# razvanmatisan/duodiff

Measured on AMD Instinct MI355X. Metric: images/sec (whole node) DuoDiff 1000-step CelebA-64, higher is better.
Workload: dtype bf16

## Files before the change

duodiff_amd/_lib.py:

```python
import ctypes as C
import os
from pathlib import Path

LIB_PATH = Path(os.environ.get("DUODIFF_LIB") or Path(__file__).resolve().parent / "libduodiff.so")

DD_OK = 0
DD_ERR_INVALID, DD_ERR_NOT_FOUND, DD_ERR_STATE, DD_ERR_HIP, DD_ERR_NOMEM, DD_ERR_UNSUPPORTED = -1, -2, -3, -4, -5, -6
DD_PREC_BF16, DD_PREC_FP32 = 0, 1
DD_VAR_BETA_TILDE, DD_VAR_BETA = 0, 1
DD_NOISE_NONE, DD_NOISE_BUFFER, DD_NOISE_PHILOX = 0, 1, 2
DD_X0_STATIC, DD_X0_DYNAMIC = 0, 1
DD_EE_MLP_PER_LAYER, DD_EE_MLP_PER_TIMESTEP, DD_EE_MLP_PER_LAYER_PER_TIMESTEP, DD_EE_ATTENTION_PROBE = 0, 1, 2, 3
ABI_VERSION = 6
DD_DEV_NO_FUSED_MLP, DD_DEV_NO_FUSED_PROJ, DD_DEV_NO_FUSED_HEAD, DD_DEV_GENERIC_EMBED, DD_DEV_MLP_EXTRAS_ONLY = 1, 2, 4, 8, 16
DD_DEV_NO_FUSED_SKIP, DD_DEV_NO_FUSED_QKV, DD_DEV_NO_FUSED_QA = 32, 64, 128
DD_PROF_DOMINANT, DD_PROF_BLOCK_TAIL, DD_PROF_FC1, DD_PROF_ROWLIN, DD_PROF_QKV_ATTENTION, DD_PROF_SPLITK = 0, 1, 2, 3, 4, 5
DD_DEV_NO_CHAINS, DD_DEV_FORCE_CHAINS, DD_DEV_NO_ROWLIN, DD_DEV_NO_ROWLIN_PROJ, DD_DEV_NO_EMBED_LN, DD_DEV_NO_SPLITK, DD_DEV_NO_ROWLIN_SKIP = 256, 512, 1024, 2048, 4096, 8192, 16384
DD_DEV_NO_SPLIT_HEADS = 32768
DD_DEV_NO_FRAG_AO, DD_DEV_NO_FRAG_SKIP, DD_DEV_NO_FRAG_X = 65536, 131072, 262144


class dd_config(C.Structure):
    _fields_ = [(n, C.c_int32) for n in (
        "img_size", "patch_size", "in_chans", "embed_dim", "depth", "num_heads", "mlp_ratio",
# ... 110 lines not shown
    "dd_bench_gemm": (C.c_int, [C.c_void_p, C.c_void_p, C.c_int, C.c_int, C.c_void_p, C.POINTER(C.c_float), C.POINTER(C.c_double)]),
    "dd_vae_create": (C.c_int, [C.c_void_p, C.c_int, C.c_int, C.POINTER(C.c_void_p)]),
    "dd_vae_set_param": (C.c_int, [C.c_void_p, C.c_char_p, C.c_void_p, C.POINTER(C.c_int64), C.c_int]),
    "dd_vae_finalize": (C.c_int, [C.c_void_p, C.c_int]),
    "dd_vae_decode": (C.c_int, [C.c_void_p, C.c_void_p, C.c_void_p, C.c_void_p, C.c_int, C.c_int, C.c_void_p]),
    "dd_vae_destroy": (None, [C.c_void_p]),
    "dd_vae_has_encoder": (C.c_int, [C.c_void_p]),
    "dd_vae_encode": (C.c_int, [C.c_void_p, C.c_void_p, C.c_void_p, C.c_void_p, C.c_void_p, C.c_void_p, C.c_int, C.c_int, C.c_void_p]),
    "dd_vae_sample": (C.c_int, [C.c_void_p, C.c_void_p, C.c_void_p, C.c_void_p, C.c_int, C.c_int, C.c_void_p]),
    "dd_profile_steps": (C.c_int, [C.c_void_p, C.c_void_p, C.c_void_p, C.c_void_p, C.c_int, C.c_int, C.c_int, C.c_void_p,
                                   C.POINTER(C.c_float), C.POINTER(C.c_int)]),
    "dd_profile_steps_chained": (C.c_int, [C.c_void_p, C.c_void_p, C.c_void_p, C.c_void_p, C.c_int, C.c_int, C.c_int, C.c_void_p,
                                           C.POINTER(C.c_float), C.POINTER(C.c_int)]),
    "dd_profile_select": (C.c_int, [C.c_void_p, C.c_int]),
    "dd_dev_qkv_attention": (C.c_int, [C.c_void_p, C.c_int, C.c_int, C.c_int, C.c_int, C.c_void_p, C.c_void_p, C.c_void_p, C.c_void_p,
                                       C.c_int, C.c_void_p, C.POINTER(C.c_float)]),
    "dd_dev_qkv_attention_rows": (C.c_int, [C.c_void_p, C.c_int, C.c_int, C.c_int, C.c_int] + [C.c_void_p] * 6 + [C.c_int, C.c_void_p, C.POINTER(C.c_float)]),
    "dd_dev_v_identity": (C.c_int, [C.c_void_p, C.c_int, C.c_int, C.c_int, C.c_int] + [C.c_void_p] * 6 + [C.c_int, C.c_void_p, C.POINTER(C.c_float)]),
    "dd_dev_v_copy": (C.c_int, [C.c_void_p] + [C.c_int] * 4 + [C.c_void_p] * 2 + [C.c_int, C.c_void_p, C.POINTER(C.c_float)]),
    "dd_dev_mlp": (C.c_int, [C.c_void_p, C.c_int, C.c_int, C.c_int, C.c_int] + [C.c_void_p] * 10 + [C.c_int, C.c_void_p, C.POINTER(C.c_float)] + [C.c_void_p] * 8),
    "dd_dev_block_tail": (C.c_int, [C.c_void_p] + [C.c_int] * 7 + [C.c_void_p] * 21 + [C.c_int, C.c_void_p, C.c_int, C.c_void_p, C.POINTER(C.c_float)]),
    "dd_dev_block_tail_frag": (C.c_int, [C.c_void_p] + [C.c_int] * 7 + [C.c_void_p] * 21 + [C.c_int, C.c_void_p, C.c_int, C.c_void_p, C.POINTER(C.c_float)] + [C.c_void_p] * 5),
    "dd_dev_qkv_attention_frag": (C.c_int, [C.c_void_p, C.c_int, C.c_int, C.c_int, C.c_int] + [C.c_void_p] * 7 + [C.c_int, C.c_void_p, C.POINTER(C.c_float)]),
    "dd_dev_head_dec": (C.c_int, [C.c_void_p] + [C.c_int] * 5 + [C.c_void_p] * 9 + [C.c_int, C.c_int, C.c_void_p, C.POINTER(C.c_float)]),
    "dd_dev_gemm": (C.c_int, [C.c_void_p] + [C.c_int] * 5 + [C.c_void_p] * 4 + [C.c_int] * 6 + [C.c_void_p] + [C.c_int] * 2 + [C.c_void_p] * 2 +
                    [C.c_int] + [C.c_void_p] * 3 + [C.c_int, C.c_int, C.c_void_p, C.POINTER(C.c_float)]),
    "dd_dev_rowlin": (C.c_int, [C.c_void_p] + [C.c_int] * 6 + [C.c_void_p] * 5 + [C.c_void_p] * 3 + [C.c_int, C.c_int, C.c_void_p, C.POINTER(C.c_float)]),
    "dd_dev_attention": (C.c_int, [C.c_void_p] + [C.c_int] * 4 + [C.c_void_p] * 4 + [C.c_int, C.c_void_p, C.POINTER(C.c_float)]),
    "dd_dev_layernorm": (C.c_int, [C.c_void_p] + [C.c_int] * 3 + [C.c_void_p] * 4 + [C.c_int] * 3 + [C.c_void_p, C.POINTER(C.c_float)]),
    "dd_dev_embed": (C.c_int, [C.c_void_p] + [C.c_int] * 9 + [C.c_void_p] * 7 + [C.c_float] + [C.c_void_p] * 3 + [C.c_int, C.c_void_p, C.POINTER(C.c_float)]),
    "dd_dev_time_mlp": (C.c_int, [C.c_void_p] + [C.c_int] * 5 + [C.c_void_p] * 6 + [C.c_float, C.c_void_p, C.c_int, C.c_void_p, C.POINTER(C.c_float)]),
    "dd_dev_vae_gather": (C.c_int, [C.c_void_p] + [C.c_int] * 6 + [C.c_void_p, C.c_void_p, C.c_size_t, C.c_void_p]),
    "dd_dev_poison_workspaces": (C.c_int, [C.c_void_p, C.c_void_p, C.c_void_p]),
    "dd_dev_graph_captures": (C.c_longlong, [C.c_void_p]),
    "dd_dev_last_sample_chains": (C.c_int, [C.c_void_p]),
    "dd_dev_set_flags": (C.c_int, [C.c_void_p, C.c_uint]),
    "dd_set_num_cus": (C.c_int, [C.c_void_p, C.c_int]),
    "dd_plan_rows": (C.c_int, [C.c_int, C.c_int, C.c_int, C.c_int, C.POINTER(C.c_int), C.POINTER(C.c_int)]),
    "dd_last_sample_timing": (C.c_int, [C.c_void_p, C.POINTER(C.c_float)]),
}

_lib = None


class EngineUnavailable(RuntimeError):
    """libduodiff.so is missing or unusable.  There is no CPU path to fall back to."""
# ... 29 lines not shown
```

duodiff_amd/csrc/attention.hip:

```cpp
#include "dd_internal.h"
#include "wave_prims.h"

#include <type_traits>
#include <utility>

namespace dd {
namespace {

constexpr int kMaxKeyTiles = 9;
constexpr int kLP = kMaxKeyTiles * 32;
constexpr int kHD = 64;
constexpr int kPartBytes = 4 * 2 * 66 * 4;

__device__ __forceinline__ int k_swz(int r) { return ((r >> 1) & 7) ^ ((r & 1) << 2); }
__device__ __forceinline__ int v_swz(int r) { return (2 * (r & 3)) ^ ((r >> 2) & 1); }

template <typename T> struct AttnLayout;
template <> struct AttnLayout<bf16_t> {
    static constexpr int kRowK = 128;
    static constexpr int kRowV = 128;
    static constexpr int kVBytes = kLP * kRowV;
};
template <> struct AttnLayout<float> {
    static constexpr int kRowK = 256 + 16;
// ... 313 lines not shown
                float f;
                if constexpr (sizeof(T) == 2) f = __builtin_amdgcn_exp2f((m[w] - M) * (0.125f * 1.4426950408889634f));
                else f = expf((m[w] - M) * 0.125f);
                num = fmaf(f, part[(w * 2 + qi) * 66 + d], num);
                den = fmaf(f, part[(w * 2 + qi) * 66 + 65], den);
            }
            out[((long long)b * L + 256 + qi) * D + hh * kHD + d] = Elem<T>::from_f32(num / den);
        }
    }
}


struct QkvAttnArgs {
    const bf16_t* h;
    const bf16_t* wimg;
    const float* bias;
    const bf16_t* hx;
    const float* xres;
    const float* ln_g;
    const float* ln_b;
    bf16_t* out;
    int B, L, H, Lp, E;
    bf16_t* out_frag = nullptr;
};

constexpr int kQaPxBytes = 8 * 6 * 2 * 32 * 4;
constexpr int kQaHxPad = 64;
constexpr int kQaHxBytes = 2 * (1024 * 2 + kQaHxPad);
constexpr int kQaAuxBytes = kQaPxBytes + kQaHxBytes + 256;
constexpr int kQaKQ = 8;
constexpr int kQaBlk = 2 * kQaKQ * 1024;
constexpr int kQaRing = 4 * kQaBlk;
static_assert(8 * 2 * 66 * 4 <= kQaPxBytes, "the split chunk's partials reuse the px area");

constexpr int qa_dma_ops(int b, int nb) { return b < nb ? 2 : 0; }
constexpr int qa_pref_ops(int b, int nb) { return (b >= 0 && b % 3 == 0 && b / 3 + 1 < nb / 3) ? kQaKQ : 0; }
constexpr int qa_younger_dma(int b, int nb) { return qa_pref_ops(b - 1, nb) + qa_dma_ops(b + 2, nb) + qa_pref_ops(b, nb); }
constexpr int qa_younger_rows(int b, int nb) { return qa_dma_ops(b, nb) + qa_dma_ops(b + 1, nb) + qa_dma_ops(b + 2, nb); }

template <int D>
__global__ void __launch_bounds__(512, 1) qkv_attention_kernel(const QkvAttnArgs a) {
    using Lay = AttnLayout<bf16_t>;
    constexpr int KS = D / 16, NS = KS / kQaKQ, NB = 3 * NS;
    static_assert(D % 128 == 0 && D >= 512 && D <= 1024, "k range in slices of 8 k-steps; hxl holds two rows of D <= 1024");
    extern __shared__ __attribute__((aligned(16))) char smem[];
    char* Ks = smem;
    char* Vt = smem + kLP * Lay::kRowK;
    float* px = reinterpret_cast<float*>(smem + kLP * Lay::kRowK + Lay::kVBytes);
    float* part = px;
    char* hxl = smem + kLP * Lay::kRowK + Lay::kVBytes + kQaPxBytes;
    char* qxl = hxl + kQaHxBytes;
    char* ring = smem + kLP * Lay::kRowK + Lay::kVBytes + kQaAuxBytes;

    int b, hh;
    if ((a.B & 7) == 0) { const int slot = blockIdx.x >> 3; b = (blockIdx.x & 7) + 8 * (slot / a.H); hh = slot % a.H; }
    else { b = blockIdx.x / a.H; hh = blockIdx.x % a.H; }
    const int tid = threadIdx.x, lane = tid & 63, wave = __builtin_amdgcn_readfirstlane(tid >> 6);
    const int half = lane >> 5, r32 = lane & 31;
    const int L = a.L, E = a.E;

    const char* wsrc = reinterpret_cast<const char*>(a.wimg) + (size_t)hh * NB * kQaBlk;
    const unsigned lane16 = lane * 16;
    auto dma_block = [&](int bb) {
#pragma unroll
        for (int i = 0; i < 2; ++i) {
            const int pc = wave * 2 + i;
            lds_dma16s(wsrc + (size_t)bb * kQaBlk + pc * 1024, lane16, ring + (bb & 3) * kQaBlk + pc * 1024);
        }
    };
    dma_block(0);
    dma_block(1);
    dma_block(2);

    const int row = 32 * wave + r32;
    const bf16x8* hfr_u = reinterpret_cast<const bf16x8*>(a.h) + ((long long)b * 8 + wave) * KS * 64;
    const bf16x8* hfr = hfr_u + lane;
    bf16x8 xs[2][kQaKQ];
#pragma unroll
    for (int ks = 0; ks < kQaKQ; ++ks) xs[0][ks] = hfr[ks * 64];

    if (a.hx) {
        for (int i = tid; i < E * (D / 8); i += 512) {
// ... 119 lines not shown
                *reinterpret_cast<uint4*>(Vt + row * 128 + (((4 * T + gp + half) ^ swv) << 4)) = uint4{s0[0], s1[0], s0[1], s1[1]};
            }
        }
    }
    __syncthreads();
    if (tid < E * 192) {
        const int e = tid / 192, c = tid % 192, j = c >> 5, col = c & 31;
        float v = a.bias ? a.bias[(j >> 1) * D + hh * kHD + 32 * (j & 1) + col] : 0.f;
#pragma unroll
        for (int kb = 0; kb < 4; ++kb) v += px[(((2 * kb + (col >> 4)) * 6 + j) * 2 + e) * 16 + (col & 15)];
        const bf16_t vb = f2bf(v);
        const int d = 32 * (j & 1) + col, r = 256 + e;
        if (j < 2) {
            *reinterpret_cast<bf16_t*>(qxl + e * 128 + d * 2) = vb;
        } else if (j < 4) {
            const int T = d >> 5, dd = d & 31, hf = (dd >> 2) & 1, ae = (dd & 3) + 4 * (dd >> 3);
            *reinterpret_cast<bf16_t*>(Ks + r * 128 + (((4 * T + 2 * hf + (ae >> 3)) ^ k_swz(r)) << 4) + (ae & 7) * 2) = vb;
        } else {
            *reinterpret_cast<bf16_t*>(Vt + r * 128 + (((d >> 3) ^ v_swz(r)) << 4) + (d & 7) * 2) = vb;
        }
    }
    __syncthreads();

    f32x4 qe[4];
    {
        const bf16_t* qrow = reinterpret_cast<const bf16_t*>(qxl) + (r32 < E ? r32 : E - 1) * kHD + 4 * half;
#pragma unroll
        for (int st = 0; st < 4; ++st) {
            const uint2 lo = *reinterpret_cast<const uint2*>(qrow + 32 * (st >> 1) + 16 * (st & 1));
            const uint2 hi = *reinterpret_cast<const uint2*>(qrow + 32 * (st >> 1) + 16 * (st & 1) + 8);
            qe[st] = __builtin_bit_cast(f32x4, uint4{lo.x, lo.y, hi.x, hi.y});
        }
    }

    {
        f32x16 o[2];
        float mx, sum;
        attend_tiles<bf16_t, 9, kMaxKeyTiles, true>(Ks, Vt, L, kMaxKeyTiles, lane, [&](int k) { return k; }, qcur, o, mx, sum);
        const float inv = 1.0f / sum;
        bf16_t* orow = a.out + ((long long)b * L + E + row) * D + hh * kHD + 8 * half;
        long long ostride = 16;
        if (a.out_frag) { orow = a.out_frag + ((((long long)b * 8 + wave) * KS + 4 * hh) * 64 + lane) * 8; ostride = 512; }
#pragma unroll
        for (int dt = 0; dt < 2; ++dt) {
            uint2 v[4];
#pragma unroll
            for (int g = 0; g < 4; ++g) {
                bf16_t v4[4];
#pragma unroll
                for (int e = 0; e < 4; ++e) v4[e] = f2bf(o[dt][4 * g + e] * inv);
                v[g] = *reinterpret_cast<const uint2*>(v4);
            }
#pragma unroll
            for (int gp = 0; gp < 4; gp += 2) {
                const auto s0 = __builtin_amdgcn_permlane32_swap(v[gp].x, v[gp + 1].x, false, false);
                const auto s1 = __builtin_amdgcn_permlane32_swap(v[gp].y, v[gp + 1].y, false, false);
                *reinterpret_cast<uint4*>(orow + (2 * dt + gp / 2) * ostride) = uint4{s0[0], s1[0], s0[1], s1[1]};
            }
        }
    }

    {
        f32x16 o[2];
        float mx, sum;
        attend_tiles<bf16_t, 9, 2, true>(Ks, Vt, L, kMaxKeyTiles, lane, [&](int k) { return k == 0 ? wave : (wave == 7 ? 8 : -1); }, qe, o, mx, sum);
        if (r32 < E) {
            float* pw = part + (wave * 2 + r32) * 66;
#pragma unroll
            for (int dt = 0; dt < 2; ++dt)
#pragma unroll
                for (int g = 0; g < 4; ++g)
                    *reinterpret_cast<f32x4*>(pw + dt * 32 + 8 * g + 4 * half) =
                        f32x4{o[dt][4 * g], o[dt][4 * g + 1], o[dt][4 * g + 2], o[dt][4 * g + 3]};
            if (half == 0) { pw[64] = mx; pw[65] = sum; }
        }
        __syncthreads();
        if (tid < E * 64) {
            const int qi = tid >> 6, d = tid & 63;
            float m[8], M = -INFINITY;
#pragma unroll
            for (int w = 0; w < 8; ++w) { m[w] = part[(w * 2 + qi) * 66 + 64]; M = fmaxf(M, m[w]); }
            float num = 0.f, den = 0.f;
#pragma unroll
            for (int w = 0; w < 8; ++w) {
                const float f = __builtin_amdgcn_exp2f((m[w] - M) * (0.125f * 1.4426950408889634f));
                num = fmaf(f, part[(w * 2 + qi) * 66 + d], num);
                den = fmaf(f, part[(w * 2 + qi) * 66 + 65], den);
            }
            a.out[((long long)b * L + qi) * D + hh * kHD + d] = f2bf(num / den);
        }
    }
}


struct VIdentityArgs {
    const bf16_t* h;
    const bf16_t* wimg;
    const float* bias;
    const float* xres;
    const float* ln_g;
    const float* ln_b;
    bf16_t* out;
    int B, L, E;
};

template <int D>
__global__ void __launch_bounds__(512, 1) v_identity_kernel(const VIdentityArgs a) {
    constexpr int KS = D / 16, NS = KS / kQaKQ, NT = D / 256;
    static_assert(D % 256 == 0 && D >= 512 && D <= 1024, "8 waves share D / 32 column tiles; a lane normalises D / 64 columns in float4s");
    extern __shared__ __attribute__((aligned(16))) char smem[];
    const int tid = threadIdx.x, lane = tid & 63, wave = __builtin_amdgcn_readfirstlane(tid >> 6);
    const int half = lane >> 5, r32 = lane & 31;
    const int L = a.L, E = a.E, n_extra = a.B * E;
// ... 136 lines not shown
    if (L == 257 || L == 258) hipLaunchKernelGGL((attention_kernel<T, 9>), dim3(B * H), dim3(256), lds, s, qkv, out, B, L, H, D, Lp);
    else hipLaunchKernelGGL((attention_kernel<T, 0>), dim3(B * H), dim3(256), lds, s, qkv, out, B, L, H, D, Lp);
    return hipGetLastError();
}

void qkv_attention_pack(int D, int H, const float* w, unsigned short (*to_bf16)(float), unsigned short* img) {
    const int NS = D / 16 / kQaKQ;
    for (int hh = 0; hh < H; ++hh)
        for (int q = 0; q < NS; ++q)
            for (int j = 0; j < 6; ++j)
                for (int ks = 0; ks < kQaKQ; ++ks)
                    pack_fragment(w, D, (j >> 1) * D + 64 * hh + 32 * (j & 1), 16 * (q * kQaKQ + ks), FRAG_K_NATURAL, to_bf16,
                                  img + ((((size_t)hh * NS + q) * 6 + j) * kQaKQ + ks) * 512);
}

bool qkv_attention_supported(int D, int H, int L, int extras) {
    return (D == 512 || D == 768 || D == 1024) && H * kHD == D && (extras == 1 || extras == 2) && L == 256 + extras;
}

static size_t v_identity_lds(int D) { return (size_t)2 * (D / 16) * 1024; }
static size_t qkv_attention_lds() { return (size_t)kLP * AttnLayout<bf16_t>::kRowK + AttnLayout<bf16_t>::kVBytes + kQaAuxBytes + kQaRing; }

hipError_t launch_qkv_attention(const bf16_t* h, const bf16_t* wimg, const float* bias, const bf16_t* hx, const float* xres,
                                const float* ln_g, const float* ln_b, bf16_t* out, int B, int L, int H, int D, int extras, hipStream_t s, bf16_t* out_frag) {
    if (!qkv_attention_supported(D, H, L, extras) || !h || !wimg || (!hx && (!xres || !ln_g || !ln_b)) || !out || B < 1) return hipErrorInvalidValue;
    const QkvAttnArgs a{h, wimg, bias, hx, xres, ln_g, ln_b, out, B, L, H, make_head_major(L, H).Lp, extras, out_frag};
    switch (D) {
        case 512: hipLaunchKernelGGL((qkv_attention_kernel<512>), dim3(B * H), dim3(512), qkv_attention_lds(), s, a); break;
        case 768: hipLaunchKernelGGL((qkv_attention_kernel<768>), dim3(B * H), dim3(512), qkv_attention_lds(), s, a); break;
        default: hipLaunchKernelGGL((qkv_attention_kernel<1024>), dim3(B * H), dim3(512), qkv_attention_lds(), s, a); break;
    }
    return hipGetLastError();
}

hipError_t launch_v_identity(const bf16_t* h, const bf16_t* wimg, const float* bias, const float* xres, const float* ln_g, const float* ln_b,
                             bf16_t* out, int B, int L, int H, int D, int extras, hipStream_t s) {
    if (!qkv_attention_supported(D, H, L, extras) || !h || !wimg || !xres || !ln_g || !ln_b || !out || B < 1) return hipErrorInvalidValue;
    const VIdentityArgs a{h, wimg, bias, xres, ln_g, ln_b, out, B, L, extras};
    const dim3 grid(B * 4 + (B * extras + 63) / 64);
    switch (D) {
        case 512: hipLaunchKernelGGL((v_identity_kernel<512>), grid, dim3(512), v_identity_lds(512), s, a); break;
        case 768: hipLaunchKernelGGL((v_identity_kernel<768>), grid, dim3(512), v_identity_lds(768), s, a); break;
        default: hipLaunchKernelGGL((v_identity_kernel<1024>), grid, dim3(512), v_identity_lds(1024), s, a); break;
    }
    return hipGetLastError();
}

template <typename T>
hipError_t launch_v_copy(const T* qkv, T* out, int B, int L, int H, int D, hipStream_t s) {
// ... 28 lines not shown
```

duodiff_amd/csrc/dd_internal.h:

```cpp
#pragma once
#include <hip/hip_runtime.h>
#include <stdint.h>

namespace dd {

typedef unsigned short bf16_t;

typedef __attribute__((ext_vector_type(8))) short bf16x8;
typedef __attribute__((ext_vector_type(4))) float f32x4;
typedef __attribute__((ext_vector_type(16))) float f32x16;
typedef unsigned u32x2 __attribute__((ext_vector_type(2)));
typedef unsigned u32x4 __attribute__((ext_vector_type(4)));

__device__ __forceinline__ bf16_t f2bf(float f) {
    __bf16 b = (__bf16)f;
    return __builtin_bit_cast(unsigned short, b);
}
__device__ __forceinline__ float bf2f(bf16_t b) {
    return __builtin_bit_cast(float, ((unsigned)b) << 16);
}

template <typename T> struct Elem;
template <> struct Elem<float> {
    static constexpr int kPerChunk = 4;
// ... 212 lines not shown
hipError_t launch_embed(const EmbedArgs& a, hipStream_t s);

struct TimeMlpArgs {
    const float *w1t, *b1, *w2t, *b2, *pos, *t_vec;
    const StepState* st;
    float* x_tok;
    int B, D, L, extras, normalize;
};
hipError_t launch_time_mlp(const TimeMlpArgs& a, hipStream_t s);

template <typename T>
hipError_t launch_layernorm(const float* x, const float* gamma, const float* beta, T* out,
                            int rows, int D, hipStream_t s);
hipError_t launch_layernorm_frag(const float* x, const float* gamma, const float* beta, bf16_t* out, bf16_t* frag, int rows, int D,
                                 int tok_l, int tok_e, hipStream_t s);

template <typename T>
hipError_t launch_attention(const T* qkv, T* out, int B, int L, int H, int D, hipStream_t s);
hipError_t init_attention_kernels();
bool qkv_attention_supported(int D, int H, int L, int extras);
void qkv_attention_pack(int D, int H, const float* w, unsigned short (*to_bf16)(float), unsigned short* img);
hipError_t launch_qkv_attention(const bf16_t* h, const bf16_t* wimg, const float* bias, const bf16_t* hx, const float* xres,
                                const float* ln_g, const float* ln_b, bf16_t* out, int B, int L, int H, int D, int extras, hipStream_t s,
                                bf16_t* out_frag = nullptr);

hipError_t launch_v_identity(const bf16_t* h, const bf16_t* wimg, const float* bias, const float* xres, const float* ln_g, const float* ln_b,
                             bf16_t* out, int B, int L, int H, int D, int extras, hipStream_t s);
template <typename T>
hipError_t launch_v_copy(const T* qkv, T* out, int B, int L, int H, int D, hipStream_t s);

struct FinalArgs {
    const float* dec;
    const float* wconv;
    const float* bconv;
    const float* x_in;
    const float* z;
    float* eps_out;
    float* x_out;
    StepState* st;
    const StepCoef* coef;
    int B, C, S, P, L, extras, noise_mode, variance;
    int advance;
    const AffineRow* atab;
    int b0 = 0;
    int layer_B = 0;
    long long w_stride = 0, b_stride = 0;
    float guide_scale = 0.f;
// ... 99 lines not shown
```

duodiff_amd/csrc/dev_harness.hip:

```cpp
#include "../../include/duodiff.h"
#include "../../include/duodiff_dev.h"
#include "engine_state.h"
#include "launch_args.h"

#include <cstring>
#include <vector>

using namespace dd;

extern "C" {

int dd_dev_mlp(dd_ctx* c, int M, int D, int hidden, int extras, const float* x_host, const float* w1, const float* b1, const float* w2,
               const float* b2, float* xres_host, unsigned short* out_host, const float* ln_in, const float* ln_out,
               unsigned short* ln_out_host, int iters, void* stream, float* ms_out, const float* ao_host, const float* wproj,
               const float* bproj, const float* skip_host, const float* wskip, const float* bskip, const float* wqkv,
               unsigned short* qkv_out_host) {
    const bool proj = ao_host && wproj && bproj;
    const bool skp = skip_host && wskip && bskip;
    const bool qk = wqkv && qkv_out_host;
    if (qk && (!proj || !ln_out || (hidden / 32) % 2)) return DD_ERR_INVALID;
    if (proj && (!ln_in || D % 128)) return DD_ERR_INVALID;
    if (skp && (!proj || !ln_out || !ln_out_host || (hidden / 32) % 2)) return DD_ERR_INVALID;
    if (!c || !x_host || !w1 || !b1 || !w2 || !b2 || !xres_host || M < 1 || iters < 0 || extras < 0 || (extras > 0 && M % (1 + extras))) return DD_ERR_INVALID;
    if (!mlp_fused_supported(D, hidden)) return ctx_fail(c, DD_ERR_UNSUPPORTED, "fused MLP: D in {64,128,256,512}, hidden % 64 == 0");
// ... 182 lines not shown
        for (int n = 0; n < 256; ++n)
            for (int k = 0; k < D; ++k)
                hf[((((size_t)b * 8 + n / 32) * (D / 16) + k / 16) * 64 + (n % 32) + 32 * ((k % 16) / 8)) * 8 + k % 8] = hb[((size_t)b * L + extras + n) * D + k];
    qkv_attention_pack(D, H, wqkv, host_f2bf, img.data());
    QkvOperands q;
    q.hf = (const bf16_t*)dev.upload(hf.data(), hf.size() * 2);
    q.img = (const bf16_t*)dev.upload(img.data(), img.size() * 2);
    if (xres_host) {
        std::vector<float> xr(M * D);
        std::memset(xr.data(), 0xFF, xr.size() * 4);
        for (int b = 0; b < B; ++b) std::memcpy(xr.data() + (size_t)b * L * D, xres_host + (size_t)b * L * D, (size_t)extras * D * 4);
        q.xres = dev.upload(xr.data(), xr.size() * 4);
        q.ln_g = dev.upload(ln, (size_t)2 * D * 4); q.ln_b = q.ln_g + D;
    } else {
        for (int b = 0; b < B; ++b) std::memset(hb.data() + ((size_t)b * L + extras) * D, 0xFF, (size_t)256 * D * 2);
        q.hx = (const bf16_t*)dev.upload(hb.data(), hb.size() * 2);
    }
    if (bqkv) q.bias = dev.upload(bqkv, (size_t)3 * D * 4);
    return q;
}

static int qkv_attention_run(dd_ctx* c, int B, int L, int H, int extras, const float* h_host, const float* wqkv, const float* bqkv,
                             const float* xres_host, const float* ln, unsigned short* out_host, unsigned short* out_frag_host, bool identity, int iters,
                             void* stream, float* ms_out) {
    if (!c || !h_host || !wqkv || !out_host || (identity ? !xres_host || !ln : xres_host && !ln) || B < 1 || iters < 0) return DD_ERR_INVALID;
    const int D = 64 * H;
    if (!qkv_attention_supported(D, H, L, extras))
        return ctx_fail(c, DD_ERR_UNSUPPORTED, std::string(identity ? "v_identity" : "qkv_attention") + ": D = 512 / 768 / 1024, L = 256 + 1 or 2 extra tokens only");
    hipStream_t s = (hipStream_t)stream;
    const size_t M = (size_t)B * L;
    DevScope dev(c);
    const QkvOperands q = qkv_operands(dev, B, L, H, extras, h_host, wqkv, bqkv, xres_host, ln);
    bf16_t* dO = dev.filled<bf16_t>((M + 8) * D * 2, 0xFF);
    const size_t pe = (size_t)B * 256 * D, guard = (size_t)8 * D;
    bf16_t* dF = out_frag_host ? dev.filled<bf16_t>((pe + 2 * guard) * 2, 0xFF) + guard : nullptr;
    auto once = [&]() {
        return identity ? launch_v_identity(q.hf, q.img, q.bias, q.xres, q.ln_g, q.ln_b, dO, B, L, H, D, extras, s)
                        : launch_qkv_attention(q.hf, q.img, q.bias, q.hx, q.xres, q.ln_g, q.ln_b, dO, B, L, H, D, extras, s, dF);
    };
    DEV_HIP(dev, once());
    DEV_HIP(dev, hipStreamSynchronize(s));
    dev.download(out_host, dO, (M + 8) * D * 2);
    if (out_frag_host) dev.download(out_frag_host, dF - guard, (pe + 2 * guard) * 2);
    DEV_HIP(dev, time_launches(s, iters, once, ms_out));
    return dev.status();
}

extern "C" {

int dd_dev_qkv_attention_rows(dd_ctx* c, int B, int L, int H, int extras, const float* h_host, const float* wqkv, const float* bqkv,
                              const float* xres_host, const float* ln, unsigned short* out_host, int iters, void* stream, float* ms_out) {
    return qkv_attention_run(c, B, L, H, extras, h_host, wqkv, bqkv, xres_host, ln, out_host, nullptr, false, iters, stream, ms_out);
}

int dd_dev_qkv_attention_frag(dd_ctx* c, int B, int L, int H, int extras, const float* h_host, const float* wqkv, const float* bqkv,
                              const float* xres_host, const float* ln, unsigned short* out_host, unsigned short* out_frag_host, int iters,
                              void* stream, float* ms_out) {
    if (!out_frag_host) return DD_ERR_INVALID;
    return qkv_attention_run(c, B, L, H, extras, h_host, wqkv, bqkv, xres_host, ln, out_host, out_frag_host, false, iters, stream, ms_out);
}

int dd_dev_v_identity(dd_ctx* c, int B, int L, int H, int extras, const float* h_host, const float* wqkv, const float* bqkv,
                      const float* xres_host, const float* ln, unsigned short* out_host, int iters, void* stream, float* ms_out) {
    return qkv_attention_run(c, B, L, H, extras, h_host, wqkv, bqkv, xres_host, ln, out_host, nullptr, true, iters, stream, ms_out);
}

int dd_dev_v_copy(dd_ctx* c, int precision, int B, int L, int H, const float* qkv_host, void* out_host, int iters, void* stream, float* ms_out) {
    const bool bf = precision == DD_PREC_BF16;
    if (!c || (!bf && precision != DD_PREC_FP32) || B < 1 || L < 1 || H < 1 || !qkv_host || !out_host || iters < 0) return DD_ERR_INVALID;
    hipStream_t s = (hipStream_t)stream;
    const int D = 64 * H;
    const size_t esz = bf ? 2 : 4, out_elems = ((size_t)B * L + 8) * D;
    const std::vector<unsigned char> img = head_major_image(bf, B, L, H, [&](size_t u, int l) { return qkv_host + (u * L + l) * 64; });
    DevScope dev(c);
    const void* dQ = dev.upload(img.data(), img.size());
    void* dO = dev.filled(out_elems * esz, 0xFF);
    auto once = [&]() {
        return bf ? launch_v_copy<bf16_t>((const bf16_t*)dQ, (bf16_t*)dO, B, L, H, D, s) : launch_v_copy<float>((const float*)dQ, (float*)dO, B, L, H, D, s);
    };
    const hipError_t first = dev.ok() ? once() : hipSuccess;
    if (first == hipErrorInvalidValue) return ctx_fail(c, DD_ERR_UNSUPPORTED, "v_copy: 1 <= L <= 288, heads of 64");
    DEV_HIP(dev, first);
// ... 306 lines not shown
```

duodiff_amd/csrc/forward.hip:

```cpp
#include "../../include/duodiff.h"
#include "../../include/duodiff_dev.h"
#include "engine_state.h"
#include "launch_args.h"

#include <cmath>

using namespace dd;

namespace dd {
Mods perturbed(const dd_pag* p, const dd_model* late) {
    Mods mo{};
    mo.pag = p; mo.pag_late = late; mo.missing = p ? nullptr : "null dd_pag";
    return mo;
}

const char* check_threshold(const dd_x0_threshold* t) {
    if (!t) return "null dd_x0_threshold";
    if (t->mode == DD_X0_STATIC) return t->range > 0.f && std::isfinite(t->range) ? nullptr : "dd_x0_threshold: range must be positive and finite";
    if (t->mode != DD_X0_DYNAMIC) return "dd_x0_threshold: unknown mode";
    if (!(t->quantile > 0.f && t->quantile <= 1.f)) return "dd_x0_threshold: quantile outside (0, 1]";
    if (!(t->s_max >= 1.f)) return "dd_x0_threshold: s_max must be at least 1 (it may be +inf)";
    return nullptr;
}
X0Threshold kernel_threshold(const dd_x0_threshold* t, long long n) {
// ... 37 lines not shown
    const WsPtrs& ws = *ch.ws;
    const int D = m->D, L = m->L, M = B * L, nb = (int)m->blocks.size();
    const int prof = c->prof_kind == DD_PROF_DOMINANT ? ((bf16 && m->fused_mlp) ? DD_PROF_BLOCK_TAIL : DD_PROF_FC1) : c->prof_kind;
    T *h = (T*)ws.h, *ao = (T*)ws.ao, *qkv = (T*)ws.qkv, *hid = (T*)ws.hid, *xb = (T*)ws.xb;
    float* ee_dec_all = ee && m->ee_batched ? (float*)ws.hid : nullptr;
    float* ee_srow_all = ee_dec_all ? ee_dec_all + (size_t)nb * M * m->pd : nullptr;
    bool ao_in_frag = false;

    int mark(int kind) {
        if (!m->time_fc1 || kind != prof) return DD_OK;
        while (m->fc1_events.size() < m->fc1_used + 1) {
            hipEvent_t e;
            DD_HIP(c, hipEventCreate(&e));
            m->fc1_events.push_back(e);
        }
        DD_HIP(c, hipEventRecord(m->fc1_events[m->fc1_used++], s));
        return DD_OK;
    }
#define DD_TIMED(kind, expr) \
    do { if (int rc_ = mark(kind)) return rc_; DD_HIP(c, expr); if (int rc_ = mark(kind)) return rc_; } while (0)

    int tile128(int N, int K, int K1) const { return bf16 && gemm_prefers_128(m->cfg.max_batch * L, N, K, K1, c->num_cus) ? 1 : 0; }
    const T* skip_of(int bi) const { return (const T*)ws.skips[nb - 1 - bi]; }
    Handoff norm1_written() const { return Handoff{!m->fused_qa, m->fused_qa}; }

    int rowlin_then_reduce(const GemmArgs<bf16_t>& g, int resid, const char* wimg, const float* ln_g, const float* ln_b, bool frag) {
        const RowLinArgs ra = rowlin_args(g, resid, wimg, ws.mlp_partial, ln_g, ln_b, (bf16_t*)h, frag ? ws.hfrag : nullptr, B, m->N, m->extras);
        DD_TIMED(DD_PROF_ROWLIN, launch_rowlin(ra, s));
        DD_HIP(c, launch_mlp_reduce(rowlin_reduce_args(ra), D, s));
        return DD_OK;
    }
    int splitk_then_reduce_ln(GemmArgs<bf16_t> g, int resid, const float* ln_g, const float* ln_b, bool frag) {
        g.partial = ws.mlp_partial; g.splits = 2;
        DD_TIMED(DD_PROF_SPLITK, launch_gemm_splitk(g, s, ch.cus));
        DD_HIP(c, launch_reduce_ln(splitk_reduce_args(g, resid, ln_g, ln_b, (bf16_t*)h, frag ? ws.hfrag : nullptr, L, m->extras), D, s));
        return DD_OK;
    }

    int embed(const float* x_img, const float* t_vec, const int64_t* y_dev, Handoff& first) {
        EmbedArgs ea{x_img, m->emb_wt, m->emb_b, m->pos, m->label, (const long long*)y_dev, t_vec, ch.st, ws.x,
                     B, m->cfg.in_chans, m->cfg.img_size, m->cfg.patch_size, D, L, m->extras,
                     m->cfg.num_classes, m->cfg.normalize_timesteps, round_up(M, 256), (c->dev_flags & DD_DEV_GENERIC_EMBED) ? 1 : 0};
        if constexpr (bf16) {
            if (m->fused_qa && !(c->dev_flags & DD_DEV_NO_EMBED_LN) && embed_ln_supported(ea)) {
                ea.ln_g = m->blocks[0].ln1_g; ea.ln_b = m->blocks[0].ln1_b; ea.ln_frag = ws.hfrag;
                first.frag = true;
// ... 62 lines not shown
        }
        DD_HIP(c, launch_gemm<T>(g, EPI_BIAS_SET, s, ch.cus));
        return DD_OK;
    }

    int norm1_attention(int bi, const Handoff& in) {
        const BlockW& w = m->blocks[bi];
        bool qa = in.frag;
        if (!in.h && !in.frag && !in.qkv) {
            if (bf16 && m->fused_qa) {
                DD_HIP(c, launch_layernorm_frag(ws.x, w.ln1_g, w.ln1_b, (bf16_t*)h, ws.hfrag, M, D, L, m->extras, s));
                qa = true;
            } else {
                DD_HIP(c, launch_layernorm<T>(ws.x, w.ln1_g, w.ln1_b, h, M, D, s));
            }
        }
        const bool masked = (pert_mask >> bi) & 1u;
        const int Bn = masked ? pert_first : B, Bi = B - Bn;
        ao_in_frag = qa && m->frag_ao && Bi == 0;
        if (qa) {
            if constexpr (bf16) {
                if (Bn > 0)
                    DD_TIMED(DD_PROF_QKV_ATTENTION, launch_qkv_attention(ws.hfrag, w.qa_img, w.qkv_b, nullptr, ws.x, w.ln1_g, w.ln1_b, (bf16_t*)ao, Bn, L, m->H, D, m->extras, s,
                                                                         ao_in_frag ? ws.aofrag : nullptr));
                if (Bi > 0)
                    DD_HIP(c, launch_v_identity(ws.hfrag + (size_t)Bn * m->N * D, w.qa_img, w.qkv_b, ws.x + (size_t)Bn * L * D, w.ln1_g, w.ln1_b,
                                                (bf16_t*)ao + (size_t)Bn * L * D, Bi, L, m->H, D, m->extras, s));
            }
            return DD_OK;
        }
        if (!in.qkv) {
            GemmArgs<T> g{h, nullptr, (const T*)w.qkv_w, w.qkv_b, nullptr, qkv, M, 3 * D, D, D, D, 0, 3 * D};
            g.hm = make_head_major(L, m->H);
            DD_HIP(c, launch_gemm<T>(g, w.qkv_b ? EPI_BIAS_STORE : EPI_STORE, s, ch.cus));
        }
        if (Bn > 0) DD_TIMED(DD_PROF_QKV_ATTENTION, launch_attention<T>(qkv, ao, Bn, L, m->H, D, s));
        if (Bi > 0)
            DD_HIP(c, launch_v_copy<T>(qkv + (size_t)Bn * 3 * D * make_head_major(L, m->H).Lp, ao + (size_t)Bn * L * D, Bi, L, m->H, D, s));
        return DD_OK;
    }

    int proj(int bi) {
        const BlockW& w = m->blocks[bi];
        GemmArgs<T> g{ao, nullptr, (const T*)w.proj_w, w.proj_b, ws.x, nullptr, M, D, D, D, D, 0, D};
        g.tile128 = tile128(D, D, D);
        if constexpr (bf16) {
            if (m->rowlin_proj) return rowlin_then_reduce(g, 1, w.rlp_img, w.ln2_g, w.ln2_b, false);
// ... 36 lines not shown
        fa.wimg = w.mlp_img; fa.b1p = w.mlp_b1p; fa.b2 = w.fc2_b;
        fa.ln_in_g = w.ln2_g; fa.ln_in_b = w.ln2_b;
        fa.xres = ws.x; fa.out = (bf16_t*)copy; fa.partial = ws.mlp_partial;
        if (m->fused_proj) { fa.ao = (const bf16_t*)ao; fa.bproj = w.proj_b; }
        if (ao_in_frag) fa.ao_frag = ws.aofrag;
        if (m->frag_skip && bi < m->half_depth) fa.out_frag = ws.skipfrags[bi];
        next.skip = m->fused_skip && bi >= m->half_depth && bi + 1 < nb;
        if (next.skip) {
            fa.skip = (const bf16_t*)skip_of(bi + 1);
            if (m->frag_skip) fa.skip_frag = ws.skipfrags[nb - 1 - (bi + 1)];
            if (ee) fa.y_tap = ws.ytap;
            fa.bskip = m->blocks[bi + 1].skip_b;
        }
        const bool h_next = bi < m->half_depth || next.skip;
        if (in.xfrag) fa.x_in_frag = ws.xfrag;
        next.xfrag = m->frag_x && h_next;
        if (next.xfrag) fa.x_out_frag = ws.xfrag;
        next.frag = m->fused_qa && h_next;
        next.qkv = !next.frag && m->fused_qkv && h_next;
        next.h = h_next && !next.frag && !next.qkv;
        if (h_next) { fa.ln_out_g = m->blocks[bi + 1].ln1_g; fa.ln_out_b = m->blocks[bi + 1].ln1_b; fa.ln_out = (bf16_t*)h; }
        if (next.frag) fa.ln_out_frag = ws.hfrag;
        if (next.qkv) { fa.qkv_out = (bf16_t*)qkv; fa.qkv_dump = ws.qkv_dump; }
        block_tail_plan(fa, B, m->N, m->extras, D, m->H, m->hidden, bi + 1 == nb);
        DD_TIMED(DD_PROF_BLOCK_TAIL, launch_mlp_fused(fa, D, s));
        DD_HIP(c, block_tail_finish(fa, D, s));
        return DD_OK;
    }

    int ee_finish() {
        if (!ee_dec_all) return DD_OK;
        FinalArgs fa = final_args(m, ch, ee_dec_all, m->heads[0].wconv, m->heads[0].bconv, nb * B);
        fa.eps_out = ee->outs;
        fa.layer_B = B; fa.w_stride = m->ee_wconv_stride; fa.b_stride = m->ee_bconv_stride;
        DD_HIP(c, launch_final(fa, s));
        if (m->ee_type != DD_EE_ATTENTION_PROBE) DD_HIP(c, launch_ee_probe_reduce(ee_srow_all, ee->cls, nb * B, L, s));
        return DD_OK;
    }

    int head() {
        const HeadW& hd = m->head;
        if (hd.wg) {
            HeadDecArgs ha{ws.x, hd.wg, hd.dc, ws.dec, M, m->pd, (L - m->extras) % 16 == 0 ? L : 0, m->extras};
            DD_HIP(c, launch_head_dec(ha, D, ch.cus, s));
            return DD_OK;
        }
        float* hf = (float*)ws.hid;
// ... 286 lines not shown
```

include/duodiff_dev.h:

```cpp
#ifndef DUODIFF_DEV_H
#define DUODIFF_DEV_H

#include "duodiff.h"
#include <stddef.h>

#ifdef __cplusplus
extern "C" {
#endif

int dd_dev_mlp(dd_ctx* ctx, int M, int D, int hidden, int extras, const float* h_host, const float* w1, const float* b1,
               const float* w2, const float* b2, float* xres_host, unsigned short* out_host, const float* ln_in,
               const float* ln_out, unsigned short* ln_out_host, int iters, void* stream, float* ms_out,
               const float* ao_host, const float* wproj, const float* bproj, const float* skip_host, const float* wskip,
               const float* bskip, const float* wqkv, unsigned short* qkv_out_host);

int dd_dev_block_tail(dd_ctx* ctx, int B, int n_patches, int extras, int D, int hidden, int last, int poison, const float* h_host,
                      const float* w1, const float* b1, const float* w2, const float* b2, const float* ln_in, const float* ao_host,
                      const float* wproj, const float* bproj, const float* ln_out, const float* skip_host, const float* wskip,
                      const float* bskip, const float* wqkv, float* xres_host, unsigned short* out_host, unsigned short* ln_out_host,
                      unsigned short* frag_host, float* tap_host, unsigned short* qkv_host, float* slab_host, int slab_rows, int* plan_out,
                      int iters, void* stream, float* ms_out);

int dd_dev_block_tail_frag(dd_ctx* ctx, int B, int n_patches, int extras, int D, int hidden, int last, int poison, const float* h_host,
                           const float* w1, const float* b1, const float* w2, const float* b2, const float* ln_in, const float* ao_host,
                           const float* wproj, const float* bproj, const float* ln_out, const float* skip_host, const float* wskip,
                           const float* bskip, const float* wqkv, float* xres_host, unsigned short* out_host, unsigned short* ln_out_host,
                           unsigned short* frag_host, float* tap_host, unsigned short* qkv_host, float* slab_host, int slab_rows, int* plan_out,
                           int iters, void* stream, float* ms_out, const unsigned short* ao_frag_host, const unsigned short* skip_frag_host,
                           const float* xin_frag_host, unsigned short* out_frag_host, float* xout_frag_host);

int dd_dev_qkv_attention(dd_ctx* ctx, int B, int L, int H, int extras, const float* h_host, const float* wqkv, const float* bqkv,
                         unsigned short* out_host, int iters, void* stream, float* ms_out);

int dd_dev_qkv_attention_rows(dd_ctx* ctx, int B, int L, int H, int extras, const float* h_host, const float* wqkv, const float* bqkv,
                              const float* xres_host, const float* ln, unsigned short* out_host, int iters, void* stream, float* ms_out);

int dd_dev_qkv_attention_frag(dd_ctx* ctx, int B, int L, int H, int extras, const float* h_host, const float* wqkv, const float* bqkv,
                              const float* xres_host, const float* ln, unsigned short* out_host, unsigned short* out_frag_host, int iters,
                              void* stream, float* ms_out);

int dd_dev_v_identity(dd_ctx* ctx, int B, int L, int H, int extras, const float* h_host, const float* wqkv, const float* bqkv,
                      const float* xres_host, const float* ln, unsigned short* out_host, int iters, void* stream, float* ms_out);

int dd_dev_v_copy(dd_ctx* ctx, int precision, int B, int L, int H, const float* qkv_host, void* out_host, int iters, void* stream,
                  float* ms_out);

int dd_dev_head_dec(dd_ctx* ctx, int M, int D, int pd, int tok_l, int tok_e, const float* x_host, const float* norm_g, const float* norm_b,
                    const float* wdec, const float* bdec, float* dec_host, const float* probe_w, const float* probe_b, float* srow_host,
                    int split, int iters, void* stream, float* ms_out);

int dd_dev_gemm(dd_ctx* ctx, int precision, int M, int N, int K, int K1, const float* A, const float* A2, const float* W, const float* bias,
                int epilogue, int tile128, int hm_L, int hm_H, int splits, int resid, const float* ln, int tok_l, int tok_e,
                float* xres_host, void* out_host, int ldo, unsigned short* h_host, unsigned short* frag_host, float* slab_host,
                int num_cus, int iters, void* stream, float* ms_out);

int dd_dev_rowlin(dd_ctx* ctx, int B, int n_patches, int extras, int K, int k_split, int set_x, const float* A, const float* A2, const float* W,
                  const float* bias, const float* ln, float* xres_host, unsigned short* x_copy_host, unsigned short* h_host, int frag,
                  int iters, void* stream, float* ms_out);

int dd_dev_attention(dd_ctx* ctx, int precision, int B, int L, int H, const float* q, const float* k, const float* v, void* out_host,
                     int iters, void* stream, float* ms_out);

// ... 46 lines not shown
```

Before: 50.29.

## Skip extra-token query attention in last block and merge extras via LDS tickets

In the fused QKV-attention kernel, the extra-token (time/label) query attention now runs before the main patch-query loop. Each wave writes its partial and takes an LDS atomic ticket, and the wave that finishes the group merges the partials. This removes a block-wide __syncthreads and the serialized merge at the end. In the last block, when the fused MLP/proj path makes the extra tokens unused, the extra-query attention is skipped entirely via a new flag, which the block-tail plan now gates on the same condition. The ticket protocol adds atomics and fence-ordering complexity and changes which wave performs the merge.

```diff
diff --git a/duodiff_amd/_lib.py b/duodiff_amd/_lib.py
--- a/duodiff_amd/_lib.py
+++ b/duodiff_amd/_lib.py
@@ -156,6 +156,7 @@
     "dd_dev_block_tail": (C.c_int, [C.c_void_p] + [C.c_int] * 7 + [C.c_void_p] * 21 + [C.c_int, C.c_void_p, C.c_int, C.c_void_p, C.POINTER(C.c_float)]),
     "dd_dev_block_tail_frag": (C.c_int, [C.c_void_p] + [C.c_int] * 7 + [C.c_void_p] * 21 + [C.c_int, C.c_void_p, C.c_int, C.c_void_p, C.POINTER(C.c_float)] + [C.c_void_p] * 5),
     "dd_dev_qkv_attention_frag": (C.c_int, [C.c_void_p, C.c_int, C.c_int, C.c_int, C.c_int] + [C.c_void_p] * 7 + [C.c_int, C.c_void_p, C.POINTER(C.c_float)]),
+    "dd_dev_qkv_attention_noq": (C.c_int, [C.c_void_p, C.c_int, C.c_int, C.c_int, C.c_int] + [C.c_void_p] * 7 + [C.c_int, C.c_void_p, C.POINTER(C.c_float)]),
     "dd_dev_head_dec": (C.c_int, [C.c_void_p] + [C.c_int] * 5 + [C.c_void_p] * 9 + [C.c_int, C.c_int, C.c_void_p, C.POINTER(C.c_float)]),
     "dd_dev_gemm": (C.c_int, [C.c_void_p] + [C.c_int] * 5 + [C.c_void_p] * 4 + [C.c_int] * 6 + [C.c_void_p] + [C.c_int] * 2 + [C.c_void_p] * 2 +
                     [C.c_int] + [C.c_void_p] * 3 + [C.c_int, C.c_int, C.c_void_p, C.POINTER(C.c_float)]),
diff --git a/duodiff_amd/csrc/attention.hip b/duodiff_amd/csrc/attention.hip
--- a/duodiff_amd/csrc/attention.hip
+++ b/duodiff_amd/csrc/attention.hip
@@ -359,12 +359,13 @@
     bf16_t* out;
     int B, L, H, Lp, E;
     bf16_t* out_frag = nullptr;
+    bool no_extra_q = false;
 };
 
 constexpr int kQaPxBytes = 8 * 6 * 2 * 32 * 4;
 constexpr int kQaHxPad = 64;
 constexpr int kQaHxBytes = 2 * (1024 * 2 + kQaHxPad);
-constexpr int kQaAuxBytes = kQaPxBytes + kQaHxBytes + 256;
+constexpr int kQaAuxBytes = kQaPxBytes + kQaHxBytes + 256 + 16;
 constexpr int kQaKQ = 8;
 constexpr int kQaBlk = 2 * kQaKQ * 1024;
 constexpr int kQaRing = 4 * kQaBlk;
@@ -374,6 +375,15 @@
 constexpr int qa_pref_ops(int b, int nb) { return (b >= 0 && b % 3 == 0 && b / 3 + 1 < nb / 3) ? kQaKQ : 0; }
 constexpr int qa_younger_dma(int b, int nb) { return qa_pref_ops(b - 1, nb) + qa_dma_ops(b + 2, nb) + qa_pref_ops(b, nb); }
 constexpr int qa_younger_rows(int b, int nb) { return qa_dma_ops(b, nb) + qa_dma_ops(b + 1, nb) + qa_dma_ops(b + 2, nb); }
+
+__device__ __forceinline__ unsigned lds_ticket(unsigned* word, int lane, unsigned add) {
+    __builtin_amdgcn_fence(__ATOMIC_RELEASE, "workgroup");
+    unsigned t = 0;
+    if (lane == 0) t = __hip_atomic_fetch_add(word, add, __ATOMIC_ACQ_REL, __HIP_MEMORY_SCOPE_WORKGROUP);
+    t = (unsigned)__builtin_amdgcn_readfirstlane((int)t);
+    __builtin_amdgcn_fence(__ATOMIC_ACQUIRE, "workgroup");
+    return t;
+}
 
 template <int D>
 __global__ void __launch_bounds__(512, 1) qkv_attention_kernel(const QkvAttnArgs a) {
@@ -387,6 +397,7 @@
     float* part = px;
     char* hxl = smem + kLP * Lay::kRowK + Lay::kVBytes + kQaPxBytes;
     char* qxl = hxl + kQaHxBytes;
+    unsigned* xq_word = reinterpret_cast<unsigned*>(qxl + 256);
     char* ring = smem + kLP * Lay::kRowK + Lay::kVBytes + kQaAuxBytes;
 
     int b, hh;
@@ -395,6 +406,7 @@
     const int tid = threadIdx.x, lane = tid & 63, wave = __builtin_amdgcn_readfirstlane(tid >> 6);
     const int half = lane >> 5, r32 = lane & 31;
     const int L = a.L, E = a.E;
+    if (tid == 0) *xq_word = 0;
 
     const char* wsrc = reinterpret_cast<const char*>(a.wimg) + (size_t)hh * NB * kQaBlk;
     const unsigned lane16 = lane * 16;
@@ -560,8 +572,23 @@
     }
     __syncthreads();
 
-    f32x4 qe[4];
-    {
+    auto merge_extras = [&]() {
+        for (int qi = 0; qi < E; ++qi) {
+            float m[8], M = -INFINITY;
+#pragma unroll
+            for (int w = 0; w < 8; ++w) { m[w] = part[(w * 2 + qi) * 66 + 64]; M = fmaxf(M, m[w]); }
+            float num = 0.f, den = 0.f;
+#pragma unroll
+            for (int w = 0; w < 8; ++w) {
+                const float f = __builtin_amdgcn_exp2f((m[w] - M) * (0.125f * 1.4426950408889634f));
+                num = fmaf(f, part[(w * 2 + qi) * 66 + lane], num);
+                den = fmaf(f, part[(w * 2 + qi) * 66 + 65], den);
+            }
+            a.out[((long long)b * L + qi) * D + hh * kHD + lane] = f2bf(num / den);
+        }
+    };
+    if (!a.no_extra_q) {
+        f32x4 qe[4];
         const bf16_t* qrow = reinterpret_cast<const bf16_t*>(qxl) + (r32 < E ? r32 : E - 1) * kHD + 4 * half;
 #pragma unroll
         for (int st = 0; st < 4; ++st) {
@@ -569,6 +596,22 @@
             const uint2 hi = *reinterpret_cast<const uint2*>(qrow + 32 * (st >> 1) + 16 * (st & 1) + 8);
             qe[st] = __builtin_bit_cast(f32x4, uint4{lo.x, lo.y, hi.x, hi.y});
         }
+        f32x16 o[2];
+        float mx, sum;
+        const int xt = (wave + 4) & 7;
+        attend_tiles<bf16_t, 9, 2, true>(Ks, Vt, L, kMaxKeyTiles, lane, [&](int k) { return k == 0 ? xt : (xt == 7 ? 8 : -1); }, qe, o, mx, sum);
+        if (r32 < E) {
+            float* pw = part + (xt * 2 + r32) * 66;
+#pragma unroll
+            for (int dt = 0; dt < 2; ++dt)
+#pragma unroll
+                for (int g = 0; g < 4; ++g)
+                    *reinterpret_cast<f32x4*>(pw + dt * 32 + 8 * g + 4 * half) =
+                        f32x4{o[dt][4 * g], o[dt][4 * g + 1], o[dt][4 * g + 2], o[dt][4 * g + 3]};
+            if (half == 0) { pw[64] = mx; pw[65] = sum; }
+        }
+        const unsigned t = lds_ticket(xq_word, lane, 1u);
+        if ((t & 15u) == 7u && t >= 16u) merge_extras();
     }
 
     {
@@ -597,36 +640,9 @@
             }
         }
     }
-
-    {
-        f32x16 o[2];
-        float mx, sum;
-        attend_tiles<bf16_t, 9, 2, true>(Ks, Vt, L, kMaxKeyTiles, lane, [&](int k) { return k == 0 ? wave : (wave == 7 ? 8 : -1); }, qe, o, mx, sum);
-        if (r32 < E) {
-            float* pw = part + (wave * 2 + r32) * 66;
-#pragma unroll
-            for (int dt = 0; dt < 2; ++dt)
-#pragma unroll
-                for (int g = 0; g < 4; ++g)
-                    *reinterpret_cast<f32x4*>(pw + dt * 32 + 8 * g + 4 * half) =
-                        f32x4{o[dt][4 * g], o[dt][4 * g + 1], o[dt][4 * g + 2], o[dt][4 * g + 3]};
-            if (half == 0) { pw[64] = mx; pw[65] = sum; }
-        }
-        __syncthreads();
-        if (tid < E * 64) {
-            const int qi = tid >> 6, d = tid & 63;
-            float m[8], M = -INFINITY;
-#pragma unroll
-            for (int w = 0; w < 8; ++w) { m[w] = part[(w * 2 + qi) * 66 + 64]; M = fmaxf(M, m[w]); }
-            float num = 0.f, den = 0.f;
-#pragma unroll
-            for (int w = 0; w < 8; ++w) {
-                const float f = __builtin_amdgcn_exp2f((m[w] - M) * (0.125f * 1.4426950408889634f));
-                num = fmaf(f, part[(w * 2 + qi) * 66 + d], num);
-                den = fmaf(f, part[(w * 2 + qi) * 66 + 65], den);
-            }
-            a.out[((long long)b * L + qi) * D + hh * kHD + d] = f2bf(num / den);
-        }
+    if (!a.no_extra_q) {
+        const unsigned t = lds_ticket(xq_word, lane, 16u);
+        if (t == 8u) merge_extras();
     }
 }
 
@@ -809,9 +825,10 @@
 static size_t qkv_attention_lds() { return (size_t)kLP * AttnLayout<bf16_t>::kRowK + AttnLayout<bf16_t>::kVBytes + kQaAuxBytes + kQaRing; }
 
 hipError_t launch_qkv_attention(const bf16_t* h, const bf16_t* wimg, const float* bias, const bf16_t* hx, const float* xres,
-                                const float* ln_g, const float* ln_b, bf16_t* out, int B, int L, int H, int D, int extras, hipStream_t s, bf16_t* out_frag) {
+                                const float* ln_g, const float* ln_b, bf16_t* out, int B, int L, int H, int D, int extras, hipStream_t s, bf16_t* out_frag,
+                                bool no_extra_q) {
     if (!qkv_attention_supported(D, H, L, extras) || !h || !wimg || (!hx && (!xres || !ln_g || !ln_b)) || !out || B < 1) return hipErrorInvalidValue;
-    const QkvAttnArgs a{h, wimg, bias, hx, xres, ln_g, ln_b, out, B, L, H, make_head_major(L, H).Lp, extras, out_frag};
+    const QkvAttnArgs a{h, wimg, bias, hx, xres, ln_g, ln_b, out, B, L, H, make_head_major(L, H).Lp, extras, out_frag, no_extra_q};
     switch (D) {
         case 512: hipLaunchKernelGGL((qkv_attention_kernel<512>), dim3(B * H), dim3(512), qkv_attention_lds(), s, a); break;
         case 768: hipLaunchKernelGGL((qkv_attention_kernel<768>), dim3(B * H), dim3(512), qkv_attention_lds(), s, a); break;
diff --git a/duodiff_amd/csrc/dd_internal.h b/duodiff_amd/csrc/dd_internal.h
--- a/duodiff_amd/csrc/dd_internal.h
+++ b/duodiff_amd/csrc/dd_internal.h
@@ -258,7 +258,7 @@
 void qkv_attention_pack(int D, int H, const float* w, unsigned short (*to_bf16)(float), unsigned short* img);
 hipError_t launch_qkv_attention(const bf16_t* h, const bf16_t* wimg, const float* bias, const bf16_t* hx, const float* xres,
                                 const float* ln_g, const float* ln_b, bf16_t* out, int B, int L, int H, int D, int extras, hipStream_t s,
-                                bf16_t* out_frag = nullptr);
+                                bf16_t* out_frag = nullptr, bool no_extra_q = false);
 
 hipError_t launch_v_identity(const bf16_t* h, const bf16_t* wimg, const float* bias, const float* xres, const float* ln_g, const float* ln_b,
                              bf16_t* out, int B, int L, int H, int D, int extras, hipStream_t s);
diff --git a/duodiff_amd/csrc/dev_harness.hip b/duodiff_amd/csrc/dev_harness.hip
--- a/duodiff_amd/csrc/dev_harness.hip
+++ b/duodiff_amd/csrc/dev_harness.hip
@@ -228,7 +228,7 @@
 
 static int qkv_attention_run(dd_ctx* c, int B, int L, int H, int extras, const float* h_host, const float* wqkv, const float* bqkv,
                              const float* xres_host, const float* ln, unsigned short* out_host, unsigned short* out_frag_host, bool identity, int iters,
-                             void* stream, float* ms_out) {
+                             void* stream, float* ms_out, bool no_extra_q = false) {
     if (!c || !h_host || !wqkv || !out_host || (identity ? !xres_host || !ln : xres_host && !ln) || B < 1 || iters < 0) return DD_ERR_INVALID;
     const int D = 64 * H;
     if (!qkv_attention_supported(D, H, L, extras))
@@ -242,7 +242,7 @@
     bf16_t* dF = out_frag_host ? dev.filled<bf16_t>((pe + 2 * guard) * 2, 0xFF) + guard : nullptr;
     auto once = [&]() {
         return identity ? launch_v_identity(q.hf, q.img, q.bias, q.xres, q.ln_g, q.ln_b, dO, B, L, H, D, extras, s)
-                        : launch_qkv_attention(q.hf, q.img, q.bias, q.hx, q.xres, q.ln_g, q.ln_b, dO, B, L, H, D, extras, s, dF);
+                        : launch_qkv_attention(q.hf, q.img, q.bias, q.hx, q.xres, q.ln_g, q.ln_b, dO, B, L, H, D, extras, s, dF, no_extra_q);
     };
     DEV_HIP(dev, once());
     DEV_HIP(dev, hipStreamSynchronize(s));
@@ -264,6 +264,12 @@
                               void* stream, float* ms_out) {
     if (!out_frag_host) return DD_ERR_INVALID;
     return qkv_attention_run(c, B, L, H, extras, h_host, wqkv, bqkv, xres_host, ln, out_host, out_frag_host, false, iters, stream, ms_out);
+}
+
+int dd_dev_qkv_attention_noq(dd_ctx* c, int B, int L, int H, int extras, const float* h_host, const float* wqkv, const float* bqkv,
+                             const float* xres_host, const float* ln, unsigned short* out_host, unsigned short* out_frag_host, int iters,
+                             void* stream, float* ms_out) {
+    return qkv_attention_run(c, B, L, H, extras, h_host, wqkv, bqkv, xres_host, ln, out_host, out_frag_host, false, iters, stream, ms_out, true);
 }
 
 int dd_dev_v_identity(dd_ctx* c, int B, int L, int H, int extras, const float* h_host, const float* wqkv, const float* bqkv,
diff --git a/duodiff_amd/csrc/forward.hip b/duodiff_amd/csrc/forward.hip
--- a/duodiff_amd/csrc/forward.hip
+++ b/duodiff_amd/csrc/forward.hip
@@ -83,6 +83,7 @@
 
     int tile128(int N, int K, int K1) const { return bf16 && gemm_prefers_128(m->cfg.max_batch * L, N, K, K1, c->num_cus) ? 1 : 0; }
     const T* skip_of(int bi) const { return (const T*)ws.skips[nb - 1 - bi]; }
+    bool extras_feed_nothing(int bi) const { return bf16 && bi + 1 == nb && m->fused_mlp && m->fused_proj; }
     Handoff norm1_written() const { return Handoff{!m->fused_qa, m->fused_qa}; }
 
     int rowlin_then_reduce(const GemmArgs<bf16_t>& g, int resid, const char* wimg, const float* ln_g, const float* ln_b, bool frag) {
@@ -191,7 +192,7 @@
             if constexpr (bf16) {
                 if (Bn > 0)
                     DD_TIMED(DD_PROF_QKV_ATTENTION, launch_qkv_attention(ws.hfrag, w.qa_img, w.qkv_b, nullptr, ws.x, w.ln1_g, w.ln1_b, (bf16_t*)ao, Bn, L, m->H, D, m->extras, s,
-                                                                         ao_in_frag ? ws.aofrag : nullptr));
+                                                                         ao_in_frag ? ws.aofrag : nullptr, extras_feed_nothing(bi)));
                 if (Bi > 0)
                     DD_HIP(c, launch_v_identity(ws.hfrag + (size_t)Bn * m->N * D, w.qa_img, w.qkv_b, ws.x + (size_t)Bn * L * D, w.ln1_g, w.ln1_b,
                                                 (bf16_t*)ao + (size_t)Bn * L * D, Bi, L, m->H, D, m->extras, s));
@@ -274,7 +275,7 @@
         if (h_next) { fa.ln_out_g = m->blocks[bi + 1].ln1_g; fa.ln_out_b = m->blocks[bi + 1].ln1_b; fa.ln_out = (bf16_t*)h; }
         if (next.frag) fa.ln_out_frag = ws.hfrag;
         if (next.qkv) { fa.qkv_out = (bf16_t*)qkv; fa.qkv_dump = ws.qkv_dump; }
-        block_tail_plan(fa, B, m->N, m->extras, D, m->H, m->hidden, bi + 1 == nb);
+        block_tail_plan(fa, B, m->N, m->extras, D, m->H, m->hidden, extras_feed_nothing(bi));
         DD_TIMED(DD_PROF_BLOCK_TAIL, launch_mlp_fused(fa, D, s));
         DD_HIP(c, block_tail_finish(fa, D, s));
         return DD_OK;
diff --git a/include/duodiff_dev.h b/include/duodiff_dev.h
--- a/include/duodiff_dev.h
+++ b/include/duodiff_dev.h
@@ -38,6 +38,10 @@
 int dd_dev_qkv_attention_frag(dd_ctx* ctx, int B, int L, int H, int extras, const float* h_host, const float* wqkv, const float* bqkv,
                               const float* xres_host, const float* ln, unsigned short* out_host, unsigned short* out_frag_host, int iters,
                               void* stream, float* ms_out);
+
+int dd_dev_qkv_attention_noq(dd_ctx* ctx, int B, int L, int H, int extras, const float* h_host, const float* wqkv, const float* bqkv,
+                             const float* xres_host, const float* ln, unsigned short* out_host, unsigned short* out_frag_host, int iters,
+                             void* stream, float* ms_out);
 
 int dd_dev_v_identity(dd_ctx* ctx, int B, int L, int H, int extras, const float* h_host, const float* wqkv, const float* bqkv,
                       const float* xres_host, const float* ln, unsigned short* out_host, int iters, void* stream, float* ms_out);
```

New measurement: 50.21. No clear change (-0.2%).
